# uci-cbcl/esm-efficient

Measured on AMD Instinct MI355X. Metric: residues/sec ESM2-650M fwd, 50k packed tokens; % bf16 MFMA peak; 1/2/4/8 GPU, higher is better.
Workload: dtype bf16

## Files before the change

### esm-efficient_amd/csrc/gemm.hip

```cpp
#include "gemm.h"
#ifndef ESME_GELU_PACKED
#define ESME_GELU_PACKED 1
#endif
#include <atomic>
#include <cstdlib>

#ifndef ESME_GEMM_P3N
#define ESME_GEMM_P3N 4
#endif
#ifndef ESME_GEMM_PERSIST_ROT
#define ESME_GEMM_PERSIST_ROT 0
#endif

namespace esme {

template <int BM, int BN, int WM, int WN, int EPI, int ROTD = 0, bool LNF = false, bool STATS = false, bool PERSIST = false, bool R32 = false, bool PAIR = false, bool F16 = false, bool RP = false>
__global__ __launch_bounds__(WM * WN * 64) void gemm_bf16_kernel(const GemmArgs a) {
    static_assert(!RP || (F16 && EPI == ESME_EPI_RESIDUAL && !R32 && !PAIR && !LNF && ROTD == 0), "pair stream: fp16 residual epilogue");
    static_assert(!F16 || ((!PAIR || (LNF && EPI == ESME_EPI_NONE)) && (EPI != ESME_EPI_RESIDUAL || R32 || RP)),
                  "fp16 operands: plain / GELU / SwiGLU epilogues, the fp32- / pair-stream residual epilogues, pair output of the LN-folded plain epilogue");
    static_assert(!LNF || EPI != ESME_EPI_RESIDUAL, "LN fold applies to the consumers of a LayerNorm");
    static_assert(!R32 || EPI == ESME_EPI_RESIDUAL, "the fp32 residual stream belongs to the residual epilogue");
    static_assert(!PAIR || (EPI != ESME_EPI_RESIDUAL && (!LNF || F16) && !STATS && !PERSIST), "(hi, lo) pair output: plain / GELU / SwiGLU epilogues of the split-operand mode; fp16: the LN-folded plain epilogue");
    static_assert(!STATS || (EPI == ESME_EPI_RESIDUAL && WTN_OK(BN, WN) && BN / WN == 64 && (WN == 2 || WN == 4)), "row statistics are emitted by the residual epilogue");
    static_assert(ROTD == 0 || (EPI == ESME_EPI_NONE && (ROTD == 16 || ROTD == 32 || ROTD == 64) && WTN_OK(BN, WN)),
                  "fused rotary: plain epilogue, head dim 16/32/64, 64-column wave tiles");
    constexpr int NW = WM * WN;
    constexpr int NT = NW * 64;
    constexpr int WTM = BM / WM, WTN = BN / WN;
    constexpr int FM = WTM / 16, FN = WTN / 16;
    constexpr int FMH = FM / 2;
    static_assert(FM % 2 == 0, "wave tile rows split in two halves");
    constexpr int A_ROWS_BYTES = BM * 128, W_ROWS_BYTES = BN * 128;
    constexpr int STAGE = A_ROWS_BYTES + W_ROWS_BYTES;
    constexpr int IA = BM * 8 / NT, IW = BN * 8 / NT;
    static_assert(BM * 8 % NT == 0 && BN * 8 % NT == 0, "tile/threads mismatch");
    static_assert(EPI != ESME_EPI_SWIGLU || WTN == 64, "swiglu needs 64-wide wave tiles");

    extern __shared__ __attribute__((aligned(16))) char smem[];
    constexpr int LDS_BYTES = 2 * (BM + BN) * 128 + ((LNF || ROTD > 0) ? BM * 12 + BN * 8 : 0) + (STATS ? WN * BM * 8 : 0) + (RP ? 2 * BN * 8 : 0);
    (void)LDS_BYTES;

    const int tid = threadIdx.x;
    const int lane = tid & 63;
    const int wave = __builtin_amdgcn_readfirstlane(tid >> 6);
    constexpr bool P8 = (NW == 8 && WM == 2 && WN == 4 && BM == 256 && BN == 256);
    const int wm = P8 ? (wave >> 2) : wave % WM, wn = P8 ? (wave & 3) : wave / WM;
    const int l15 = lane & 15, lq = lane >> 4;
    ESME_TRACE_REAL(8);
    ESME_TRACE_MARK(0);

#ifdef ESME_GEMM_TRACE
    if (a.stagger > 0 && blockIdx.x < 256) {
        const int n = (blockIdx.x * a.stagger) >> 8;
        for (int i = 0; i < n; ++i) __builtin_amdgcn_s_sleep(16);
    }
#endif
    unsigned int pid, pid_end = 0u, pid_step = 0u;
    if constexpr (PERSIST) {
        const unsigned int nblk = (unsigned int)(a.tiles_m * a.tiles_n);
        const unsigned int q = nblk >> 3, r = nblk & 7u, xcd = blockIdx.x & 7u, slot = blockIdx.x >> 3;
        const unsigned int base = (xcd < r) ? xcd * (q + 1) : r * (q + 1) + (xcd - r) * q;
        pid_step = gridDim.x >> 3;
        pid = base + slot;
        pid_end = base + q + (xcd < r ? 1u : 0u);
        if (pid >= pid_end) return;
    } else {
        pid = xcd_remap(blockIdx.x, gridDim.x);
    }
    int64_t m0;
    int n0;
    auto tile_coords = [&](const unsigned int id) {
        const int per_band = a.gm * a.tiles_n;
        const int band = id / per_band, lb = id - band * per_band;
        const int rows = min(a.gm, a.tiles_m - band * a.gm);
        const int grp = rows * a.gn;
        const int ng = lb / grp, rg = lb - ng * grp;
        const int tile_n = ng * a.gn + rg / rows;
        const int64_t tile_m = (int64_t)band * a.gm + rg % rows;
        m0 = tile_m * BM;
        n0 = tile_n * BN;
    };
    tile_coords(pid);

    const u16* srcA[IA];
    const u16* srcW[IW];
    auto set_sources = [&]() {
        int ln = lane;
        if constexpr (PERSIST) asm volatile("" : "+v"(ln));
#pragma unroll
        for (int i = 0; i < IA; ++i) {
            const int q = (i * NW + wave) * 64 + ln;
            const int row = q >> 3, c = (q & 7) ^ ((row >> 1) & 7);
            const int trow = P8 ? ((row >> 6) & 1) * WTM + (row >> 7) * (WTM / 2) + (row & 63) : row;
            int64_t gr = m0 + trow;
            gr = gr < a.M ? gr : a.M - 1;
            srcA[i] = a.A + gr * a.lda + c * 8;
        }
#pragma unroll
        for (int i = 0; i < IW; ++i) {
            const int q = (i * NW + wave) * 64 + ln;
            const int row = q >> 3, c = (q & 7) ^ ((row >> 1) & 7);
            const int tcol = P8 ? ((row >> 5) & 3) * WTN + (row >> 7) * (WTN / 2) + (row & 31) : row;
            int gr = n0 + tcol;
            gr = gr < a.N ? gr : a.N - 1;
            srcW[i] = a.W + (int64_t)gr * (a.kt_wrap > 0 ? a.kt_wrap * BK : a.K) + c * 8;
        }
    };
    set_sources();

    auto w_k0 = [&](const int kt) { return ((a.kt_wrap > 0 && kt >= a.kt_wrap) ? kt - a.kt_wrap : kt) * BK; };
    auto stage = [&](int kt, int buf) {
        char* base = smem + buf * STAGE;
        const int k0 = kt * BK, k0w = w_k0(kt);
#pragma unroll
        for (int i = 0; i < IA; ++i)
            __builtin_amdgcn_global_load_lds((gptr_t)(srcA[i] + k0), (lptr_t)(base + (i * NW + wave) * 1024), 16, 0, 0);
#pragma unroll
        for (int i = 0; i < IW; ++i)
            __builtin_amdgcn_global_load_lds((gptr_t)(srcW[i] + k0w),
                                             (lptr_t)(base + A_ROWS_BYTES + (i * NW + wave) * 1024), 16, 0, 0);
    };

    const int swz = (l15 >> 1) & 7;
    int coff[2];
#pragma unroll
    for (int ks = 0; ks < 2; ++ks) coff[ks] = ((ks * 4 + lq) ^ swz) << 4;
    const int rowA = (P8 ? wm * (WTM / 2) + l15 : wm * WTM + l15) * 128;
    const int rowW = A_ROWS_BYTES + (P8 ? wn * (WTN / 2) + l15 : wn * WTN + l15) * 128;

    f32x4 acc[FN][FM];
#pragma unroll
    for (int i = 0; i < FN; ++i)
#pragma unroll
        for (int j = 0; j < FM; ++j)
#pragma unroll
            for (int r = 0; r < 4; ++r) acc[i][j][r] = 0.f;

    const int KT = a.K / BK;
    struct FragW { bf16x8 v[FN]; };
    struct FragA { bf16x8 v[FMH]; };
    auto rdW = [&](FragW& f, const char* base, int ks) {
#pragma unroll
        for (int i = 0; i < FN; ++i) f.v[i] = *reinterpret_cast<const bf16x8*>(base + rowW + i * 16 * 128 + coff[ks]);
    };
    auto rdA = [&](FragA& f, const char* base, int ks, int h) {
#pragma unroll
        for (int j = 0; j < FMH; ++j) f.v[j] = *reinterpret_cast<const bf16x8*>(base + rowA + (h * FMH + j) * 16 * 128 + coff[ks]);
    };
    static_assert(IA % 2 == 0 && IW % 2 == 0, "the LDS-DMA pieces of a K-tile split in two halves");
    constexpr int NP = IA + IW;
    auto stage_piece = [&](int kt, int buf, int p) {
        char* base = smem + buf * STAGE;
        const int k0 = kt * BK;
        ESME_LDS_CHECK(p < IA ? base + (p * NW + wave) * 1024 : base + A_ROWS_BYTES + ((p - IA) * NW + wave) * 1024, 1024, smem, 2 * STAGE);
        if (p < IA) __builtin_amdgcn_global_load_lds((gptr_t)(srcA[p] + k0), (lptr_t)(base + (p * NW + wave) * 1024), 16, 0, 0);
        else __builtin_amdgcn_global_load_lds((gptr_t)(srcW[p - IA] + w_k0(kt)),
                                              (lptr_t)(base + A_ROWS_BYTES + ((p - IA) * NW + wave) * 1024), 16, 0, 0);
    };
    f32x2* lnst = reinterpret_cast<f32x2*>(smem + 2 * STAGE);
    int* lpos = reinterpret_cast<int*>(smem + 2 * STAGE + BM * 8);
    f32x4* c1s = reinterpret_cast<f32x4*>(smem + 2 * STAGE + BM * 12);
    f32x4* c2s = c1s + BN / 4;
    constexpr bool ROT32 = PAIR && ROTD > 0;
    constexpr int CPRW = ROTD > 0 ? (ROT32 ? ROTD / 4 : ROTD / 8) : 1;
    constexpr int TB = (ROT32 ? 4 : 2) * ROTD;
    constexpr int TAB_INSTR = WTM * CPRW / 64;
    constexpr int TAB_PER_WAVE = (TAB_INSTR + WN - 1) / WN;
    auto rot_prefetch = [&](int fb, int h) {
        if constexpr (ROTD > 0) {
            if (n0 >= a.rot_cols) return;
            char* tab = smem + fb * STAGE + wm * (WTM * TB);
#pragma unroll
            for (int it = 0; it < TAB_PER_WAVE; ++it) {
                if ((it & 1) != h && TAB_PER_WAVE > 1) continue;
                if (TAB_PER_WAVE == 1 && h != 0) continue;
                const int g = wn * TAB_PER_WAVE + it;
                if (g >= TAB_INSTR) continue;
                const int idx = g * 64 + lane;
                const int r = idx / CPRW;
                const int c = (idx % CPRW) ^ (r & (CPRW - 1));
                const int p = lpos[wm * WTM + r];
                const void* src;
                if constexpr (ROT32) src = (c < CPRW / 2) ? reinterpret_cast<const float*>(a.cosT) + (int64_t)p * ROTD + c * 4
                                                          : reinterpret_cast<const float*>(a.sinT) + (int64_t)p * ROTD + (c - CPRW / 2) * 4;
                else src = (c < CPRW / 2) ? a.cosT + (int64_t)p * ROTD + c * 8
                                          : a.sinT + (int64_t)p * ROTD + (c - CPRW / 2) * 8;
                ESME_LDS_CHECK(tab + g * 1024, 1024, smem, 2 * STAGE);
                __builtin_amdgcn_global_load_lds((gptr_t)src, (lptr_t)(tab + g * 1024), 16, 0, 0);
            }
        }
    };
    f32x4* pscale = reinterpret_cast<f32x4*>(smem + 2 * STAGE + (STATS ? WN * BM * 8 : 0));
    int sp = 0;
    auto fill_scales = [&](const int half) {
        if constexpr (RP) {
            if (tid < BN / 4) {
                int n = n0 + tid * 4;
                n = n < a.N - 4 ? n : a.N - 4;
                const f32x4 one = {1.f, 1.f, 1.f, 1.f};
                ESME_LDS_CHECK(&pscale[half * (BN / 2) + BN / 4 + tid], 16, smem, LDS_BYTES);
                pscale[half * (BN / 2) + tid] = a.ps_in ? *reinterpret_cast<const f32x4*>(a.ps_in + n) : one;
                pscale[half * (BN / 2) + BN / 4 + tid] = a.ps_out ? *reinterpret_cast<const f32x4*>(a.ps_out + n) : one;
            }
        }
    };
    int par = 0;
    stage(0, 0);
    auto make_strips = [&]() {
        if constexpr (ROTD > 0) {
            if (tid < BM) {
                int64_t m = m0 + tid;
                m = m < a.M ? m : a.M - 1;
                int p = a.pos[m];
                lpos[tid] = p < a.max_len ? p : a.max_len - 1;
            }
        }
        if constexpr (LNF) {
            if (tid < BM) {
                int64_t m = m0 + tid;
                m = m < a.M ? m : a.M - 1;
                float s1 = 0.f, s2 = 0.f;
                const f32x2* pp = reinterpret_cast<const f32x2*>(a.ln_partial) + m;
                const int n256 = (a.K + 255) >> 8;
                if (a.ln_nblk > n256) {
                    int b = 0;
                    for (; b + 10 <= a.ln_nblk; b += 10) {
                        f32x2 p[10];
    #pragma unroll
                        for (int u = 0; u < 10; ++u) p[u] = pp[(int64_t)(b + u) * a.stat_ld];
    #pragma unroll
                        for (int u = 0; u < 10; u += 2) { s1 += p[u][0] + p[u + 1][0]; s2 += p[u][1] + p[u + 1][1]; }
                    }
                    for (; b + 2 <= a.ln_nblk; b += 2) {
                        const f32x2 p0 = pp[(int64_t)b * a.stat_ld], p1 = pp[(int64_t)(b + 1) * a.stat_ld];
                        s1 += p0[0] + p1[0]; s2 += p0[1] + p1[1];
                    }
                    if (b < a.ln_nblk) { const f32x2 p = pp[(int64_t)b * a.stat_ld]; s1 += p[0]; s2 += p[1]; }
                } else {
                    int b = 0;
                    for (; b + 10 <= a.ln_nblk; b += 10) {
                        f32x2 p[10];
    #pragma unroll
                        for (int u = 0; u < 10; ++u) p[u] = pp[(int64_t)(b + u) * a.stat_ld];
    #pragma unroll
                        for (int u = 0; u < 10; ++u) { s1 += p[u][0]; s2 += p[u][1]; }
                    }
                    for (; b + 5 <= a.ln_nblk; b += 5) {
                        f32x2 p[5];
    #pragma unroll
                        for (int u = 0; u < 5; ++u) p[u] = pp[(int64_t)(b + u) * a.stat_ld];
    #pragma unroll
                        for (int u = 0; u < 5; ++u) { s1 += p[u][0]; s2 += p[u][1]; }
                    }
                    for (; b < a.ln_nblk; ++b) {
                        const f32x2 p = pp[(int64_t)b * a.stat_ld];
                        s1 += p[0]; s2 += p[1];
                    }
                }
                if (a.ovf && !(s2 < 3.0e38f)) atomicOr(a.ovf, 1);
                const float inv = 1.0f / (float)a.ln_dim;
                const float mean = s1 * inv;
                const float rstd = rsqrtf(fmaxf(s2 * inv - mean * mean, 0.f) + a.ln_eps);
                ESME_LDS_CHECK(&lnst[tid], 8, smem, LDS_BYTES);
                lnst[tid] = f32x2{rstd, rstd * mean};
            }
            if (tid < BN / 4) {
                int n = n0 + tid * 4;
                n = n < a.N - 4 ? n : a.N - 4;
                ESME_LDS_CHECK(&c2s[tid], 16, smem, LDS_BYTES);
                c1s[tid] = *reinterpret_cast<const f32x4*>(a.ln_c1 + n);
                c2s[tid] = *reinterpret_cast<const f32x4*>(a.ln_c2 + n);
            }
        }

    };
    make_strips();
    fill_scales(0);
    __syncthreads();
    FragW w0;
    FragA a0, a1;
#ifdef ESME_GEMM_TRACE
    unsigned long long trace_barrier_wait = 0, trace_vm_wait = 0;
    int trace_tile = -1;
#endif
    for (;;) {
    ESME_TRACE_MARK(1);
#ifdef ESME_GEMM_TRACE
    ++trace_tile;
#endif
    if constexpr (PERSIST) set_sources();
    if constexpr (P8) {
    if (KT > 1) {
        stage_piece(1, par ^ 1, IA); stage_piece(1, par ^ 1, IA + 1);
        stage_piece(1, par ^ 1, 0); stage_piece(1, par ^ 1, 1);
        stage_piece(1, par ^ 1, IA + 2); stage_piece(1, par ^ 1, IA + 3);
    }
    ESME_TRACE_SEAM(27, 2);
    if (wm == 1) __builtin_amdgcn_s_barrier();
    bf16x8 fa[FMH][2], fw[FN][2];
    constexpr int HALFB = (BM / 2) * 128;
    static_assert(FN == 4 && FMH == 4, "P8 geometry");
    auto rdW2 = [&](const char* base) {
#pragma unroll
        for (int i = 0; i < FN; ++i)
#pragma unroll
            for (int ks = 0; ks < 2; ++ks) {
                ESME_LDS_CHECK(base + rowW + (i >> 1) * HALFB + (i & 1) * 16 * 128 + coff[ks], 16, smem, 2 * STAGE);
                fw[i][ks] = *reinterpret_cast<const bf16x8*>(base + rowW + (i >> 1) * HALFB + (i & 1) * 16 * 128 + coff[ks]);
            }
    };
    auto rdAh = [&](const char* base, const int h) {
#pragma unroll
        for (int f = 0; f < FMH; ++f)
#pragma unroll
            for (int ks = 0; ks < 2; ++ks) {
                ESME_LDS_CHECK(base + rowA + h * HALFB + f * 16 * 128 + coff[ks], 16, smem, 2 * STAGE);
                fa[f][ks] = *reinterpret_cast<const bf16x8*>(base + rowA + h * HALFB + f * 16 * 128 + coff[ks]);
            }
    };
    auto mma = [&](const int j0) {
        asm volatile("s_waitcnt lgkmcnt(0)" ::: "memory");
        __builtin_amdgcn_sched_barrier(0);
        __builtin_amdgcn_s_barrier();
        __builtin_amdgcn_sched_barrier(0);
#pragma unroll
        for (int ks = 0; ks < 2; ++ks)
#pragma unroll
            for (int i = 0; i < FN; ++i)
#pragma unroll
                for (int f = 0; f < FMH; ++f)
                    acc[i][j0 + f] = mfma_16x16x32<F16>(fw[i][ks], fa[f][ks], acc[i][j0 + f]);
        __builtin_amdgcn_sched_barrier(0);
        __builtin_amdgcn_s_barrier();
        __builtin_amdgcn_sched_barrier(0);
    };
    for (int kt = 0; kt < KT; ++kt) {
        const int buf = (kt + par) & 1;
        const char* base = smem + buf * STAGE;
        const bool m1 = kt + 1 < KT, m2 = kt + 2 < KT;
        rdW2(base);
        rdAh(base, 0);
        if (m1) { stage_piece(kt + 1, buf ^ 1, 2); stage_piece(kt + 1, buf ^ 1, 3); }
        else rot_prefetch(buf ^ 1, 0);
        if (kt == 0) ESME_TRACE_SEAM(28, 2);
        mma(0);
        if (kt == 0) ESME_TRACE_SEAM(29, 2);
        rdAh(base, 1);
        if (m2) {
            stage_piece(kt + 2, buf, IA); stage_piece(kt + 2, buf, IA + 1);
            stage_piece(kt + 2, buf, 0); stage_piece(kt + 2, buf, 1);
            stage_piece(kt + 2, buf, IA + 2); stage_piece(kt + 2, buf, IA + 3);
        } else if (!m1) rot_prefetch(buf ^ 1, 1);
#ifdef ESME_GEMM_TRACE
        const unsigned long long bw0 = __builtin_readcyclecounter();
#endif
        if (m2) asm volatile("s_waitcnt vmcnt(6)" ::: "memory");
        else asm volatile("s_waitcnt vmcnt(0)" ::: "memory");
#ifdef ESME_GEMM_TRACE
        trace_vm_wait += __builtin_readcyclecounter() - bw0;
#endif
        mma(FMH);
    }
    ESME_TRACE_SEAM(16, 1);
    if (wm == 0) __builtin_amdgcn_s_barrier();
    ESME_TRACE_SEAM(17, 1);
    } else {
    rdW(w0, smem + par * STAGE, 0);
    rdA(a0, smem + par * STAGE, 0, 0);
    constexpr int P3 = (NP * ESME_GEMM_P3N) / 8;
    static_assert(FMH >= 2, "activation reads need FMH - 1 of every FMH MFMA slots");
    using std::integral_constant;
    auto sub = [&](FragW& w, const FragA& ca, auto H, auto NEWW, FragA& na, const char* nbase, const int nks,
                   const int nh, const bool rd_on, const bool on, const int kt, const int buf, auto PF, auto PL) {
        constexpr int h = decltype(H)::value, pf = decltype(PF)::value, pl = decltype(PL)::value, cnt = pl - pf, total = FN * FMH;
        constexpr bool neww = decltype(NEWW)::value;
        int na_next = 0;
#pragma unroll
        for (int m = 0; m < total; ++m) {
            const int i = m / FMH, j = m % FMH;
            acc[i][h * FMH + j] = mfma_16x16x32<F16>(w.v[i], ca.v[j], acc[i][h * FMH + j]);
            if (neww && j == FMH - 1) {
                if (rd_on) { ESME_LDS_CHECK(nbase + rowW + i * 16 * 128 + coff[nks], 16, smem, 2 * STAGE); w.v[i] = *reinterpret_cast<const bf16x8*>(nbase + rowW + i * 16 * 128 + coff[nks]); }
            } else if (na_next < FMH) {
                if (rd_on) { ESME_LDS_CHECK(nbase + rowA + (nh * FMH + na_next) * 16 * 128 + coff[nks], 16, smem, 2 * STAGE); na.v[na_next] = *reinterpret_cast<const bf16x8*>(nbase + rowA + (nh * FMH + na_next) * 16 * 128 + coff[nks]); }
                ++na_next;
            }
#pragma unroll
            for (int q = 0; q < (cnt > 0 ? cnt : 0); ++q)
                if (m == (q * total) / (cnt > 0 ? cnt : 1) && on) stage_piece(kt, buf, pf + q);
            __builtin_amdgcn_sched_barrier(0);
        }
    };
    using I0 = integral_constant<int, 0>; using I1 = integral_constant<int, 1>;
    using YES = integral_constant<bool, true>; using NO = integral_constant<bool, false>;
    if (KT > 1) {
#pragma unroll
        for (int p = 0; p < P3; ++p) stage_piece(1, par ^ 1, p);
    }
    for (int kt = 0; kt < KT; ++kt) {
        const int buf = (kt + par) & 1;
        const char* base = smem + buf * STAGE;
        const bool more = kt + 1 < KT, more2 = kt + 2 < KT;
        if (!more) rot_prefetch(buf ^ 1, 0);
        __builtin_amdgcn_sched_barrier(0);
        sub(w0, a0, I0{}, NO{}, a1, base, 0, 1, true, more, kt + 1, buf ^ 1, integral_constant<int, P3>{}, integral_constant<int, NP>{});
        if (!more) rot_prefetch(buf ^ 1, 1);
        __builtin_amdgcn_sched_barrier(0);
        sub(w0, a1, I1{}, YES{}, a0, base, 1, 0, true, false, 0, 0, I0{}, I0{});
        sub(w0, a0, I0{}, NO{}, a1, base, 1, 1, true, false, 0, 0, I0{}, I0{});
#ifdef ESME_GEMM_TRACE
        const unsigned long long bw0 = __builtin_readcyclecounter();
        asm volatile("s_waitcnt vmcnt(0) lgkmcnt(0)" ::: "memory");
        const unsigned long long bw1 = __builtin_readcyclecounter();
        trace_vm_wait += bw1 - bw0;
#endif
        __syncthreads();
#ifdef ESME_GEMM_TRACE
        trace_barrier_wait += __builtin_readcyclecounter() - bw1;
#endif
        __builtin_amdgcn_sched_barrier(0);
        sub(w0, a1, I1{}, YES{}, a0, smem + (buf ^ 1) * STAGE, 0, 0, more, more2, kt + 2, buf, I0{}, integral_constant<int, P3>{});
    }
    }
    ESME_TRACE_MARK(2);
#ifdef ESME_GEMM_TRACE
    if (a.trace && threadIdx.x == 0) { a.trace[(size_t)blockIdx.x * ESME_TRACE_STRIDE + 10] = trace_barrier_wait; a.trace[(size_t)blockIdx.x * ESME_TRACE_STRIDE + 11] = trace_vm_wait; }
#endif
#ifdef ESME_GEMM_TRACE
    if (a.nt_store == 3) return;
#endif

    int lane_e = threadIdx.x & 63;
    asm volatile("" : "+v"(lane_e));
    const int l15 = lane_e & 15, lq = lane_e >> 4, lane = lane_e;
    constexpr int OUTC = (EPI == ESME_EPI_SWIGLU) ? WTN / 2 : WTN;
    constexpr int CH = OUTC / 8;
    constexpr int ROWB = OUTC * 2;
    constexpr int RPI = 64 / CH;
    constexpr int NPASS = RP ? (BM == 256 ? 4 : 1)
                             : ((R32 && BM == 256) ? 4 : ((PERSIST || (PAIR && BM == 256)) ? 2 : 1));
    constexpr int RPP = WTM / NPASS;
    constexpr int FMP = FM / NPASS;
    static_assert(!PERSIST || (FM % 2 == 0), "two-pass epilogue");
    const int lastbuf = (a.K / BK - 1 + par) & 1;
    char* slab = smem + (PERSIST ? lastbuf * STAGE : 0) + wave * (RPP * ROWB) * (RP ? 2 : 1);
    const int64_t em0 = m0;
    const int en0 = n0;
    const int n_out = (EPI == ESME_EPI_SWIGLU) ? (a.N >> 1) : a.N;
    const int nw0 = (EPI == ESME_EPI_SWIGLU) ? ((n0 + wn * WTN) >> 1) : (n0 + wn * WTN);
    const int64_t mw0 = m0 + wm * WTM;
    auto slab_off = [&](const int r, const int cl) { return r * ROWB + (((cl >> 3) ^ (r & (CH - 1))) << 4) + (((cl >> 2) & 1) << 3); };

    if constexpr (LNF) {
        f32x2 st[FM];
#pragma unroll
        for (int j = 0; j < FM; ++j) st[j] = lnst[wm * WTM + j * 16 + l15];
#pragma unroll
        for (int i = 0; i < FN; ++i) {
            const int q4 = (wn * WTN + i * 16 + 4 * lq) >> 2;
            const f32x4 c1q = c1s[q4], c2q = c2s[q4];
#pragma unroll
            for (int j = 0; j < FM; ++j) {
#pragma unroll
                for (int e = 0; e < 4; ++e)
                    acc[i][j][e] = fmaf(st[j][0], acc[i][j][e], fmaf(-st[j][1], c1q[e], c2q[e]));
            }
        }
    }

    if constexpr (ROTD > 0) {
#pragma unroll
        for (int i = 0; i < FN; ++i) {
            if (LNF || !a.bias) continue;
            const u32x2 bw = *reinterpret_cast<const u32x2*>(a.bias + nw0 + i * 16 + 4 * lq);
            const float b0 = bf_lo(bw[0]), b1 = bf_hi(bw[0]), b2 = bf_lo(bw[1]), b3 = bf_hi(bw[1]);
#pragma unroll
            for (int j = 0; j < FM; ++j) {
                acc[i][j][0] += b0; acc[i][j][1] += b1; acc[i][j][2] += b2; acc[i][j][3] += b3;
            }
        }
        const char* tab = smem + (lastbuf ^ 1) * STAGE + wm * (WTM * TB);
        if (nw0 < a.rot_cols) {
#pragma unroll
            for (int j = 0; j < FM; ++j) {
                const int r = j * 16 + l15;
                const char* trow = tab + r * TB + (ROT32 ? 0 : (lq & 1) * 8);
                if constexpr (ROTD == 16) {
                    float cv[4], sv[4];
                    if constexpr (ROT32) {
                        const f32x4 cq = *reinterpret_cast<const f32x4*>(trow + (((lq & 1) ^ (r & 3)) << 4));
                        const f32x4 sq = *reinterpret_cast<const f32x4*>(trow + (((2 + (lq & 1)) ^ (r & 3)) << 4));
#pragma unroll
                        for (int e = 0; e < 4; ++e) { cv[e] = cq[e]; sv[e] = sq[e]; }
                    } else {
                        const u32x2 cw = *reinterpret_cast<const u32x2*>(trow + ((0 ^ (r & 1)) << 4));
                        const u32x2 sw = *reinterpret_cast<const u32x2*>(trow + ((1 ^ (r & 1)) << 4));
                        cv[0] = lo16<F16>(cw[0]); cv[1] = hi16<F16>(cw[0]); cv[2] = lo16<F16>(cw[1]); cv[3] = hi16<F16>(cw[1]);
// ... 289 lines not shown
#pragma unroll
                        for (int e = 0; e < 4; ++e) o[e] = gelu_erf<GELU_DEG>(o[e]);
#endif
                    }
                    if constexpr (R32) {
                        const int n = nw0 + cl;
                        const int64_t m = mw0 + pass * RPP + r;
#pragma unroll
                        for (int e = 0; e < 4; ++e) o[e] = fmaf(a.alpha, o[e], xr[i][jj][e]);
                        if (m < a.M && n < a.N) store_stream(reinterpret_cast<f32x4*>(a.resid32 + m * a.ld32 + n), f32x4{o[0], o[1], o[2], o[3]}, a.stream_out);
                    } else if constexpr (EPI == ESME_EPI_RESIDUAL) {
                        const u32x2 rw = *reinterpret_cast<const u32x2*>(slab + slab_off(r, cl));
                        o[0] = bf_lo(rw[0]) + a.alpha * o[0]; o[1] = bf_hi(rw[0]) + a.alpha * o[1];
                        o[2] = bf_lo(rw[1]) + a.alpha * o[2]; o[3] = bf_hi(rw[1]) + a.alpha * o[3];
                    }
                }
                u32x2 pk = {pack16<F16>(o[0], o[1]), pack16<F16>(o[2], o[3])};
                if (PAIR && half == 0) {
                    acc[i][j][0] = o[0] - lo16<F16>(pk[0]); acc[i][j][1] = o[1] - hi16<F16>(pk[0]);
                    acc[i][j][2] = o[2] - lo16<F16>(pk[1]); acc[i][j][3] = o[3] - hi16<F16>(pk[1]);
                }
                ESME_LDS_CHECK(slab + slab_off(r, cl), 8, smem, 2 * STAGE);
                *reinterpret_cast<u32x2*>(slab + slab_off(r, cl)) = pk;
            }
            if constexpr (EPI == ESME_EPI_RESIDUAL && !R32) __builtin_amdgcn_sched_barrier(0);
        }
        if (pass + 1 < NPASS && half == NHALF - 1) load_x32(pass + 1);
        __builtin_amdgcn_wave_barrier();
        ESME_TRACE_MARK(5);
        if constexpr (PERSIST) {
            if (pass == NPASS / 2 - 1) {
                ESME_TRACE_SEAM(19, 1);
                __syncthreads();
                ESME_TRACE_SEAM(20, 1);
                pid += pid_step;
                have_next = pid < pid_end;
                if (have_next) {
                    tile_coords(pid);
                    set_sources();
                    par = lastbuf ^ 1;
                    stage(0, par);
                    make_strips();
                }
                ESME_TRACE_SEAM(21, 1);
            }
        }
        if constexpr (PERSIST) {
            if (pass == 0) ESME_TRACE_SEAM(31, 1);
            if (pass == NPASS - 1) ESME_TRACE_SEAM(23, 1);
            if (pass == NPASS - 1 && have_next) asm volatile("s_waitcnt vmcnt(0)" ::: "memory");
            if (pass == NPASS - 1) ESME_TRACE_SEAM(24, 1);
        }
        const int rl = lane / CH, ch = lane % CH;
        const int n = nw0 + ch * 8;
        const bool col_ok = n < n_out && !(PAIR && half == 1 && a.pair_cols > 0 && en0 >= a.pair_cols);
        constexpr bool QKG = F16 && LNF && ROTD > 0 && !PAIR;
        const bool qk_guard = QKG && a.qk_sumsq != nullptr && nw0 < a.rot_cols;
        float qk_max = 0.f;
        unsigned int* qk_slot = nullptr;
        unsigned int qk_cur = 0u;
        if constexpr (QKG) {
            if (qk_guard && lane < 8 && (n % ROTD) == 0 && n < a.rot_cols) {
                const int ea = a.rot_cols >> 1;
                qk_slot = a.qk_sumsq + (n >= ea ? ea / ROTD : 0) + (n % ea) / ROTD;
                qk_cur = *qk_slot;
            }
        }
        if (col_ok || STATS) {
#pragma unroll
        for (int gsel = 0; gsel < (QKG ? 2 : 1); ++gsel) {
            if (QKG && (gsel == 1) != qk_guard) continue;
#pragma unroll
            for (int it = 0; it < RPP / RPI; ++it) {
                const int r = it * RPI + rl;
                const int64_t m = mw0 + pass * RPP + r;
                ESME_LDS_CHECK(slab + r * ROWB + ((ch ^ (r & (CH - 1))) << 4), 16, smem, 2 * STAGE);
                const u32x4 v = *reinterpret_cast<const u32x4*>(slab + r * ROWB + ((ch ^ (r & (CH - 1))) << 4));
                if (col_ok && m < a.M && ESME_TUNE_STORE_OK) store_stream(reinterpret_cast<u32x4*>(a.C + m * a.ldc + n + (PAIR ? half * a.pair_off : 0)), v, a.stream_out);
                if (QKG && gsel == 1) {
                    float ss = sumsq8_f16(v);
                    ss += dpp_f32<0xB1>(ss);
                    if constexpr (ROTD >= 32) ss += dpp_f32<0x4E>(ss);
                    if constexpr (ROTD == 64) ss += dpp_f32<0x141>(ss);
                    qk_max = fmaxf(qk_max, ss);
                }
                if constexpr (STATS) {
                    float f[8];
                    unpack8t<F16>(v, f);
                    float t1 = ((f[0] + f[1]) + (f[2] + f[3])) + ((f[4] + f[5]) + (f[6] + f[7]));
                    float t2 = ((f[0] * f[0] + f[1] * f[1]) + (f[2] * f[2] + f[3] * f[3])) +
                               ((f[4] * f[4] + f[5] * f[5]) + (f[6] * f[6] + f[7] * f[7]));
                    t1 += dpp_f32<0xB1>(t1); t2 += dpp_f32<0xB1>(t2);
                    t1 += dpp_f32<0x4E>(t1); t2 += dpp_f32<0x4E>(t2);
                    t1 += dpp_f32<0x141>(t1); t2 += dpp_f32<0x141>(t2);
                    ESME_LDS_CHECK(&blkst[wn * BM + wm * WTM + pass * RPP + r], 8, smem, LDS_BYTES);
                    if (ch == 0) blkst[wn * BM + wm * WTM + pass * RPP + r] = col_ok ? f32x2{t1, t2} : f32x2{0.f, 0.f};
                }
            }
        }
        }
        if constexpr (QKG) {
            if (qk_guard) {
                qk_max = lanes8_max_f32(qk_max);
                if (qk_slot && __float_as_uint(qk_max) > qk_cur) atomicMax(qk_slot, __float_as_uint(qk_max));
            }
        }
        if constexpr (PERSIST) { if (pass == 0) ESME_TRACE_SEAM(22, 1); else ESME_TRACE_SEAM(25, 1); }
        }
        }
        }
        ESME_TRACE_MARK(6);
        if constexpr (STATS) {
            asm volatile("s_waitcnt lgkmcnt(0)" ::: "memory");
            __builtin_amdgcn_s_barrier();
            if (tid < BM && em0 + tid < a.M) {
                f32x2 acc2 = blkst[tid];
                acc2[0] += blkst[BM + tid][0]; acc2[1] += blkst[BM + tid][1];
                if constexpr (WN == 4) {
                    f32x2 hi2 = blkst[2 * BM + tid];
                    hi2[0] += blkst[3 * BM + tid][0]; hi2[1] += blkst[3 * BM + tid][1];
                    acc2[0] += hi2[0]; acc2[1] += hi2[1];
                }
                *reinterpret_cast<f32x2*>(a.stats_out + 2 * ((int64_t)(en0 / BN) * a.stat_ld + em0 + tid)) = acc2;
            }
        }
        ESME_TRACE_MARK(7);
        ESME_TRACE_REAL(9);
    } else {
        if constexpr (EPI != ESME_EPI_SWIGLU) {
    #pragma unroll
            for (int i = 0; i < FN; ++i) {
                const int n = nw0 + i * 16 + 4 * lq;
    #pragma unroll
                for (int j = 0; j < FM; ++j) {
                    const int64_t m = mw0 + j * 16 + l15;
                    if (m >= a.M) continue;
    #pragma unroll
                    for (int e = 0; e < 4; ++e) {
                        if (n + e < a.N) {
                            float v = acc[i][j][e] + ((a.bias && ROTD == 0 && !LNF) ? bf2f(a.bias[n + e]) : 0.f);
                            if constexpr (EPI == ESME_EPI_GELU) v = gelu_erf<LNF ? ESME_GELU_DEG : 7>(v);
                            if constexpr (R32) { float* xp = a.resid32 + m * a.ld32 + n + e; v = fmaf(a.alpha, v, *xp); *xp = v; }
                            else if constexpr (EPI == ESME_EPI_RESIDUAL) v = bf2f(a.resid[m * a.ldr + n + e]) + a.alpha * v;
                            if (a.c32) a.c32[m * a.ldc32 + n + e] = v;
                            else a.C[m * a.ldc + n + e] = f2h<F16>(v);
                        }
                    }
                }
            }
        }
    }
    if constexpr (!PERSIST) {
        break;
    } else {
        if (!have_next) break;
#pragma unroll
        for (int i = 0; i < FN; ++i)
#pragma unroll
            for (int j = 0; j < FM; ++j)
#pragma unroll
                for (int r = 0; r < 4; ++r) acc[i][j][r] = 0.f;
        asm volatile("s_waitcnt lgkmcnt(0)" ::: "memory");
        ESME_TRACE_SEAM(26, 1);
        __builtin_amdgcn_s_barrier();
    }
    }
}
// ... 91 lines not shown
                    case 32: return lnf ? ESME_LH(ESME_EPI_NONE, 32, true, false, false) : fail(ESME_ERR_UNSUPPORTED, "gemm: fp16 fused rotary runs LayerNorm-folded only");
                    case 64: return lnf ? ESME_LH(ESME_EPI_NONE, 64, true, false, false) : fail(ESME_ERR_UNSUPPORTED, "gemm: fp16 fused rotary runs LayerNorm-folded only");
                    default: return fail(ESME_ERR_UNSUPPORTED, "gemm: fused rotary needs head dim 16, 32 or 64");
                }
            case ESME_EPI_GELU: return lnf ? ESME_LH(ESME_EPI_GELU, 0, true, false, false) : ESME_LH(ESME_EPI_GELU, 0, false, false, false);
            case ESME_EPI_SWIGLU: return lnf ? ESME_LH(ESME_EPI_SWIGLU, 0, true, false, false) : fail(ESME_ERR_UNSUPPORTED, "gemm: fp16 SwiGLU runs LayerNorm-folded only");
            case ESME_EPI_RESIDUAL:
                if (a.pair_off)
                    return stats ? launch_one<BM, BN, WM, WN, ESME_EPI_RESIDUAL, 0, false, true, false, false, false, true, true>(a, s)
                                 : launch_one<BM, BN, WM, WN, ESME_EPI_RESIDUAL, 0, false, false, false, false, false, true, true>(a, s);
                return stats ? ESME_LH(ESME_EPI_RESIDUAL, 0, false, true, true) : ESME_LH(ESME_EPI_RESIDUAL, 0, false, false, true);
            default: return fail(ESME_ERR_ARG, "gemm: unknown epilogue");
        }
#undef ESME_LH
    }
    switch (epi) {
        case ESME_EPI_NONE:
            switch (rotd) {
                case 0: return lnf ? ESME_L(ESME_EPI_NONE, 0, true, false) : ESME_L(ESME_EPI_NONE, 0, false, false);
                case 16: return lnf ? ESME_L(ESME_EPI_NONE, 16, true, false) : ESME_L(ESME_EPI_NONE, 16, false, false);
                case 32: return lnf ? ESME_L(ESME_EPI_NONE, 32, true, false) : ESME_L(ESME_EPI_NONE, 32, false, false);
                case 64: return lnf ? ESME_L(ESME_EPI_NONE, 64, true, false) : ESME_L(ESME_EPI_NONE, 64, false, false);
                default: return fail(ESME_ERR_UNSUPPORTED, "gemm: fused rotary needs head dim 16, 32 or 64");
            }
        case ESME_EPI_GELU: return lnf ? ESME_L(ESME_EPI_GELU, 0, true, false) : ESME_L(ESME_EPI_GELU, 0, false, false);
        case ESME_EPI_SWIGLU: return lnf ? ESME_L(ESME_EPI_SWIGLU, 0, true, false) : ESME_L(ESME_EPI_SWIGLU, 0, false, false);
        case ESME_EPI_RESIDUAL:
            if (a.resid32) return stats ? launch_one<BM, BN, WM, WN, ESME_EPI_RESIDUAL, 0, false, true, false, true>(a, s)
                                        : launch_one<BM, BN, WM, WN, ESME_EPI_RESIDUAL, 0, false, false, false, true>(a, s);
            return stats ? ESME_L(ESME_EPI_RESIDUAL, 0, false, true) : ESME_L(ESME_EPI_RESIDUAL, 0, false, false);
        default: return fail(ESME_ERR_ARG, "gemm: unknown epilogue");
    }
#undef ESME_L
}

}

using namespace esme;

static int esme::cu_count() {
    static std::atomic<int> cached[64];
    int dev = 0;
    (void)hipGetDevice(&dev);
    int v = cached[dev & 63].load(std::memory_order_relaxed);
    if (v <= 0) {
        if (hipDeviceGetAttribute(&v, hipDeviceAttributeMultiprocessorCount, dev) != hipSuccess || v <= 0) v = 256;
        cached[dev & 63].store(v, std::memory_order_relaxed);
    }
    return v;
}
#ifdef ESME_GEMM_TRACE
extern "C" void esme_hip_debug_set_gemm_nt(int v) { esme::g_nt_store = v; }
extern "C" void esme_hip_debug_set_gemm_stagger(int v) { esme::g_stagger = v; }
static unsigned long long* g_trace = nullptr;
extern "C" void esme_hip_debug_set_gemm_trace(void* p) { g_trace = (unsigned long long*)p; }
#endif

static int pick_tile(int64_t M, int N, const esme_gemm_opts_t* opts) {
    if (opts && opts->tile) return opts->tile;
    const int64_t big_tiles = ((M + 255) / 256) * ((N + 255) / 256);
    return (N >= 256 && big_tiles >= 160) ? 2 : 1;
}

extern "C" int esme_hip_gemm_stats_blocks_opts(int64_t M, int N, const esme_gemm_opts_t* opts) {
    const int bn = pick_tile(M, N, opts) == 2 ? 256 : 128;
    return (N + bn - 1) / bn;
}
extern "C" int esme_hip_gemm_stats_blocks(int64_t M, int N) { return esme_hip_gemm_stats_blocks_opts(M, N, nullptr); }

extern "C" int esme_hip_gemm_bf16_opts(const void* A, int64_t lda, const void* W, const void* bias, const void* resid,
                                       int64_t ldr, void* C, int64_t ldc, int64_t M, int N, int K, int epilogue,
                                       float alpha, const esme_gemm_fusion_t* fu, const esme_gemm_opts_t* opts, void* stream) {
    ESME_CHECK_ARG(!opts || (opts->struct_bytes == (int)sizeof(esme_gemm_opts_t) && opts->tile >= 0 && opts->tile <= 2),
                   "gemm: options struct of another ABI or bad tile");
    ESME_CHECK_ARG(M >= 0 && N > 0 && K > 0, "gemm: bad sizes");
    ESME_CHECK_ARG(epilogue >= ESME_EPI_NONE && epilogue <= ESME_EPI_SWIGLU, "gemm: unknown epilogue");
    if (M == 0) return ESME_OK;
    ESME_CHECK_ARG(A && W && C, "gemm: null pointer");
    if (K % BK != 0) ESME_FAIL(ESME_ERR_UNSUPPORTED, "gemm: K must be a multiple of 64");
    const int n_out = epilogue == ESME_EPI_SWIGLU ? N / 2 : N;
    if (epilogue == ESME_EPI_SWIGLU && N % 64 != 0) ESME_FAIL(ESME_ERR_UNSUPPORTED, "gemm: swiglu needs N % 64 == 0");
    ESME_CHECK_ARG(lda >= K && lda % 8 == 0 && ldc >= n_out, "gemm: bad lda/ldc");
    ESME_CHECK_ARG(aligned16(A) && aligned16(W), "gemm: A and W must be 16-byte aligned");
    ESME_CHECK_ARG(!bias || (reinterpret_cast<uintptr_t>(bias) & 7u) == 0, "gemm: misaligned bias");
    int vec_ok = (ldc % 8 == 0) && aligned16(C) && (n_out % 8 == 0) && N >= 8;
    const bool r32 = fu && fu->resid32;
    if (r32) {
        ESME_CHECK_ARG(epilogue == ESME_EPI_RESIDUAL, "gemm: resid32 belongs to the residual epilogue");
        ESME_CHECK_ARG(fu->ld32 >= N && fu->ld32 % 4 == 0 && aligned16(fu->resid32), "gemm: resid32 needs ld32 >= N, ld32 % 4 == 0, 16-byte alignment");
        if (!vec_ok) ESME_FAIL(ESME_ERR_UNSUPPORTED, "gemm: the fp32 residual stream needs a 16-byte addressable C and N % 8 == 0");
    } else if (epilogue == ESME_EPI_RESIDUAL) {
        ESME_CHECK_ARG(resid && ldr >= N, "gemm: residual epilogue needs resid with ldr >= N");
        vec_ok = vec_ok && (ldr % 8 == 0) && aligned16(resid) && N >= 8;
    }
    if (epilogue == ESME_EPI_SWIGLU && !vec_ok) ESME_FAIL(ESME_ERR_UNSUPPORTED, "gemm: swiglu needs ldc % 8 == 0 and a 16-byte aligned C");
    GemmArgs a{(const u16*)A, lda, (const u16*)W, (const u16*)bias, (const u16*)resid, ldr, (u16*)C, ldc, M, N, K, alpha, 0, vec_ok,
               nullptr, nullptr, nullptr, 0, 0, 0, 1, 1, 0, 0, nullptr, 0, 0, 0.f, nullptr, nullptr, nullptr};
#ifdef ESME_GEMM_TRACE
    a.nt_store = g_nt_store; a.stagger = g_stagger; a.trace = g_trace;
#endif
    if (opts) { a.opt_gm = opts->raster_gm; a.opt_gn = opts->raster_gn; a.opt_persist = opts->persist; }
    int rotd = 0;
    bool lnf = false, stats = false;
    if (r32) { a.resid32 = fu->resid32; a.ld32 = fu->ld32; }
    ESME_CHECK_ARG(!fu || (!fu->pair_scale_in && !fu->pair_scale_out && !fu->ext_off) || (fu->f16 && fu->pair_off && epilogue == ESME_EPI_RESIDUAL),
                   "gemm: pair_scale_in / pair_scale_out / ext_* belong to the fp16 pair stream's residual epilogue");
    ESME_CHECK_ARG(!fu || !fu->pair_cols || (fu->f16 && fu->pair_off && epilogue == ESME_EPI_NONE), "gemm: pair_cols belongs to the fp16 pair output");
    ESME_CHECK_ARG(!fu || !fu->col_absmax || (fu->f16 && fu->pair_off && epilogue == ESME_EPI_RESIDUAL), "gemm: col_absmax belongs to the fp16 pair stream's residual epilogue");
    ESME_CHECK_ARG(!fu || !fu->qk_sumsq || (fu->f16 && fu->ln_partial && fu->head_dim != 0 && !fu->pair_off), "gemm: qk_sumsq belongs to the fp16 LN-folded projection with fused rotary (single output)");
    if (fu && fu->f16 && fu->pair_off && epilogue == ESME_EPI_NONE) {
        ESME_CHECK_ARG(fu->ln_partial && !r32 && !fu->w_k && !fu->c32 && !fu->stats_out, "gemm: the fp16 pair output belongs to the LN-folded plain epilogue");
        ESME_CHECK_ARG(fu->pair_off >= N && fu->pair_off % 8 == 0 && ldc >= fu->pair_off + (fu->pair_cols > 0 ? fu->pair_cols : N) && fu->pair_cols >= 0 && fu->pair_cols % 256 == 0,
                       "gemm: pair_off must be a multiple of 8 with N <= pair_off and room for the lo columns; pair_cols a multiple of 256");
        if (!vec_ok) ESME_FAIL(ESME_ERR_UNSUPPORTED, "gemm: pair output needs a 16-byte addressable C and N % 8 == 0");
        a.pair_off = fu->pair_off; a.pair_cols = fu->pair_cols;
    } else if (fu && fu->f16 && fu->pair_off) {
        ESME_CHECK_ARG(epilogue == ESME_EPI_RESIDUAL && !r32 && !fu->w_k && !fu->c32 && !fu->ln_partial, "gemm: the fp16 pair stream belongs to the residual epilogue");
        ESME_CHECK_ARG(fu->pair_off >= N && fu->pair_off % 8 == 0 && ldc >= fu->pair_off + N && ldr >= fu->pair_off + N,
                       "gemm: pair_off must be a multiple of 8 with N <= pair_off <= ldc - N, ldr - N");
        if (!vec_ok) ESME_FAIL(ESME_ERR_UNSUPPORTED, "gemm: the pair stream needs 16-byte addressable rows and N % 8 == 0");
        a.pair_off = fu->pair_off;
        ESME_CHECK_ARG((!fu->pair_scale_in || aligned16(fu->pair_scale_in)) && (!fu->pair_scale_out || aligned16(fu->pair_scale_out)) && (N % 4 == 0),
                       "gemm: pair_scale_in / pair_scale_out must be 16-byte aligned float (N) vectors");
        a.ps_in = fu->pair_scale_in; a.ps_out = fu->pair_scale_out;
        if (fu->ext_off) {
            ESME_CHECK_ARG(fu->ext_off >= N && fu->ext_off + 64 <= fu->pair_off && fu->ext_n >= 0 && fu->ext_n <= 64 && (fu->ext_n == 0 || fu->ext_sel),
                           "gemm: the extension tile is 64 columns between hi and lo (N <= ext_off, ext_off + 64 <= pair_off) with <= 64 selected columns");
            a.ext_sel = fu->ext_sel; a.ext_n = fu->ext_n; a.ext_off = fu->ext_off;
        }
        ESME_CHECK_ARG(!fu->col_absmax || (reinterpret_cast<uintptr_t>(fu->col_absmax) & 3u) == 0, "gemm: misaligned col_absmax");
        a.col_absmax = fu->col_absmax;
    } else if (fu && (fu->w_k || fu->pair_off || fu->c32)) {
        if (fu->w_k) {
            ESME_CHECK_ARG(fu->w_k > 0 && fu->w_k % BK == 0 && (K == fu->w_k || K == 2 * fu->w_k), "gemm: w_k (the K of W) must be a multiple of 64 with K = w_k or K = 2 w_k (the K-tile index of W wraps once)");
            if (fu->w_k < K) a.kt_wrap = fu->w_k / BK;
        }
        if (fu->pair_off) {
            ESME_CHECK_ARG(epilogue != ESME_EPI_RESIDUAL && !fu->ln_partial && !fu->stats_out, "gemm: pair output belongs to the plain / GELU / SwiGLU epilogues without LN fold");
            ESME_CHECK_ARG(fu->pair_off >= n_out && fu->pair_off % 8 == 0 && ldc >= fu->pair_off + n_out, "gemm: pair_off must be a multiple of 8 with n_out <= pair_off <= ldc - n_out");
            if (!vec_ok) ESME_FAIL(ESME_ERR_UNSUPPORTED, "gemm: pair output needs a 16-byte addressable C and N % 8 == 0");
            a.pair_off = fu->pair_off;
        }
        if (fu->c32) {
            ESME_CHECK_ARG(!fu->pair_off && epilogue != ESME_EPI_SWIGLU && fu->ldc32 >= N && (reinterpret_cast<uintptr_t>(fu->c32) & 3u) == 0, "gemm: c32 needs ldc32 >= N, no pair output, no SwiGLU");
            a.c32 = fu->c32; a.ldc32 = fu->ldc32;
            a.vec_ok = 0;
        }
    }
    if (fu && fu->f16) {
        ESME_CHECK_ARG(!fu->w_k && !fu->c32 && (!fu->pair_off || epilogue == ESME_EPI_RESIDUAL || epilogue == ESME_EPI_NONE), "gemm: fp16 operands do not combine with the split-operand fields");
        ESME_CHECK_ARG(epilogue != ESME_EPI_RESIDUAL || r32 || fu->pair_off, "gemm: fp16 operands run the residual epilogue on the fp32 stream or the fp16 pair stream");
        if (!vec_ok) ESME_FAIL(ESME_ERR_UNSUPPORTED, "gemm: fp16 operands need a 16-byte addressable C and N % 8 == 0");
        a.f16 = 1;
    }
    if (fu) {
        if (fu->head_dim != 0) {
            ESME_CHECK_ARG(epilogue == ESME_EPI_NONE, "gemm: fused rotary needs ESME_EPI_NONE");
            ESME_CHECK_ARG(fu->cos && fu->sin && fu->pos && fu->max_len > 0, "gemm: fused rotary needs cos, sin, pos, max_len");
            if (fu->head_dim != 16 && fu->head_dim != 32 && fu->head_dim != 64)
                ESME_FAIL(ESME_ERR_UNSUPPORTED, "gemm: fused rotary needs head dim 16, 32 or 64 (use esme_hip_rotary_varlen otherwise)");
            if (N % 64 != 0 || fu->rot_cols % 64 != 0 || fu->rot_cols < 0 || fu->rot_cols > N || !vec_ok)
                ESME_FAIL(ESME_ERR_UNSUPPORTED, "gemm: fused rotary needs N, rot_cols multiples of 64, rot_cols <= N, 16-byte addressable C");
            ESME_CHECK_ARG(aligned16(fu->cos) && aligned16(fu->sin), "gemm: misaligned rotary tables");
            ESME_CHECK_ARG(!fu->pair_off || fu->q_scale == 0.f, "gemm: q_scale does not combine with a pair output");
            a.cosT = (const u16*)fu->cos; a.sinT = (const u16*)fu->sin; a.pos = fu->pos;
            a.max_len = fu->max_len; a.rot_cols = fu->rot_cols;
// ... 88 lines not shown
```

Baseline: 826,800.

## Stage GEMM tiles with buffer_load LDS DMA using scalar row offsets

Result: slower. 817,400, median of 2 (-1.1%).

```diff
diff --git a/esm-efficient_amd/csrc/gemm.hip b/esm-efficient_amd/csrc/gemm.hip
--- a/esm-efficient_amd/csrc/gemm.hip
+++ b/esm-efficient_amd/csrc/gemm.hip
@@ -3,6 +3,7 @@
 #define ESME_GELU_PACKED 1
 #endif
 #include <atomic>
+#include <type_traits>
 #include <cstdlib>
 
 #ifndef ESME_GEMM_P3N
@@ -83,43 +84,59 @@
     };
     tile_coords(pid);
 
-    const u16* srcA[IA];
-    const u16* srcW[IW];
+    static_assert(NW % 2 == 0, "chunk swizzle independent of the piece index");
+    const unsigned int ldA = (unsigned int)a.lda * 2u, ldW = (unsigned int)(a.kt_wrap > 0 ? a.kt_wrap * BK : a.K) * 2u;
+    unsigned int voffA, voffW;
+    {
+        const unsigned int r = (unsigned int)lane >> 3, c = ((unsigned int)lane & 7u) ^ ((((unsigned int)wave & 1u) << 2) + ((unsigned int)lane >> 4));
+        voffA = r * ldA + c * 16u;
+        voffW = r * ldW + c * 16u;
+    }
+    auto rowA_of = [&](const int i) { return P8 ? (i & 1) * WTM + (i >> 1) * (WTM / 2) + wave * 8 : (i * NW + wave) * 8; };
+    auto rowW_of = [&](const int i) { return P8 ? ((i & 1) * 2 + (wave >> 2)) * WTN + (i >> 1) * (WTN / 2) + (wave & 3) * 8 : (i * NW + wave) * 8; };
+    auto make_rsrc = [&](const u16* p, const unsigned int bytes) -> u32x4 {
+        const uint64_t v = (uint64_t)(uintptr_t)p;
+        return u32x4{(unsigned int)__builtin_amdgcn_readfirstlane((int)(unsigned int)v),
+                     (unsigned int)__builtin_amdgcn_readfirstlane((int)((unsigned int)(v >> 32) & 0xffffu)),
+                     (unsigned int)__builtin_amdgcn_readfirstlane((int)bytes), 0x00020000u};
+    };
+    u32x4 rsA, rsW;
     auto set_sources = [&]() {
-        int ln = lane;
-        if constexpr (PERSIST) asm volatile("" : "+v"(ln));
-#pragma unroll
-        for (int i = 0; i < IA; ++i) {
-            const int q = (i * NW + wave) * 64 + ln;
-            const int row = q >> 3, c = (q & 7) ^ ((row >> 1) & 7);
-            const int trow = P8 ? ((row >> 6) & 1) * WTM + (row >> 7) * (WTM / 2) + (row & 63) : row;
-            int64_t gr = m0 + trow;
-            gr = gr < a.M ? gr : a.M - 1;
-            srcA[i] = a.A + gr * a.lda + c * 8;
-        }
-#pragma unroll
-        for (int i = 0; i < IW; ++i) {
-            const int q = (i * NW + wave) * 64 + ln;
-            const int row = q >> 3, c = (q & 7) ^ ((row >> 1) & 7);
-            const int tcol = P8 ? ((row >> 5) & 3) * WTN + (row >> 7) * (WTN / 2) + (row & 31) : row;
-            int gr = n0 + tcol;
-            gr = gr < a.N ? gr : a.N - 1;
-            srcW[i] = a.W + (int64_t)gr * (a.kt_wrap > 0 ? a.kt_wrap * BK : a.K) + c * 8;
-        }
+        const int64_t mrows = a.M - m0;
+        const unsigned int vm = mrows < BM ? (unsigned int)mrows : (unsigned int)BM;
+        const int ncols = a.N - n0;
+        const unsigned int vn = ncols < BN ? (unsigned int)ncols : (unsigned int)BN;
+        rsA = make_rsrc(a.A + m0 * a.lda, (vm - 1u) * ldA + (unsigned int)a.K * 2u);
+        rsW = make_rsrc(a.W + (int64_t)n0 * (ldW >> 1), vn * ldW);
     };
     set_sources();
+    auto dma16 = [&](const u32x4 rs, const unsigned int voff, const unsigned int soff, const char* dst, auto FRESH) {
+        const unsigned int d = (unsigned int)__builtin_amdgcn_readfirstlane((int)(unsigned int)(uintptr_t)dst);
+        const unsigned int so = (unsigned int)__builtin_amdgcn_readfirstlane((int)soff);
+        const u32x4 r = {(unsigned int)__builtin_amdgcn_readfirstlane((int)rs[0]), (unsigned int)__builtin_amdgcn_readfirstlane((int)rs[1]),
+                         (unsigned int)__builtin_amdgcn_readfirstlane((int)rs[2]), 0x00020000u};
+        unsigned int keep;
+#if defined(ESME_DEBUG_LDS) || defined(ESME_GEMM_TRACE)
+        constexpr bool pad = true;
+#else
+        constexpr bool pad = decltype(FRESH)::value;
+#endif
+        if constexpr (pad)
+            asm volatile("s_nop 4\n\ts_mov_b32 %0, m0\n\ts_mov_b32 m0, %2\n\ts_nop 0\n\tbuffer_load_dwordx4 %1, %3, %4 offen lds\n\ts_mov_b32 m0, %0"
+                         : "=&s"(keep) : "v"(voff), "s"(d), "s"(r), "s"(so) : "memory");
+        else
+            asm volatile("s_mov_b32 %0, m0\n\ts_mov_b32 m0, %2\n\ts_nop 0\n\tbuffer_load_dwordx4 %1, %3, %4 offen lds\n\ts_mov_b32 m0, %0"
+                         : "=&s"(keep) : "v"(voff), "s"(d), "s"(r), "s"(so) : "memory");
+    };
 
     auto w_k0 = [&](const int kt) { return ((a.kt_wrap > 0 && kt >= a.kt_wrap) ? kt - a.kt_wrap : kt) * BK; };
     auto stage = [&](int kt, int buf) {
         char* base = smem + buf * STAGE;
-        const int k0 = kt * BK, k0w = w_k0(kt);
-#pragma unroll
-        for (int i = 0; i < IA; ++i)
-            __builtin_amdgcn_global_load_lds((gptr_t)(srcA[i] + k0), (lptr_t)(base + (i * NW + wave) * 1024), 16, 0, 0);
-#pragma unroll
-        for (int i = 0; i < IW; ++i)
-            __builtin_amdgcn_global_load_lds((gptr_t)(srcW[i] + k0w),
-                                             (lptr_t)(base + A_ROWS_BYTES + (i * NW + wave) * 1024), 16, 0, 0);
+        const unsigned int k0 = (unsigned int)(kt * BK) * 2u, k0w = (unsigned int)w_k0(kt) * 2u;
+#pragma unroll
+        for (int i = 0; i < IA; ++i) dma16(rsA, voffA, (unsigned int)rowA_of(i) * ldA + k0, base + (i * NW + wave) * 1024, std::true_type{});
+#pragma unroll
+        for (int i = 0; i < IW; ++i) dma16(rsW, voffW, (unsigned int)rowW_of(i) * ldW + k0w, base + A_ROWS_BYTES + (i * NW + wave) * 1024, std::true_type{});
     };
 
     const int swz = (l15 >> 1) & 7;
@@ -152,11 +169,9 @@
     constexpr int NP = IA + IW;
     auto stage_piece = [&](int kt, int buf, int p) {
         char* base = smem + buf * STAGE;
-        const int k0 = kt * BK;
         ESME_LDS_CHECK(p < IA ? base + (p * NW + wave) * 1024 : base + A_ROWS_BYTES + ((p - IA) * NW + wave) * 1024, 1024, smem, 2 * STAGE);
-        if (p < IA) __builtin_amdgcn_global_load_lds((gptr_t)(srcA[p] + k0), (lptr_t)(base + (p * NW + wave) * 1024), 16, 0, 0);
-        else __builtin_amdgcn_global_load_lds((gptr_t)(srcW[p - IA] + w_k0(kt)),
-                                              (lptr_t)(base + A_ROWS_BYTES + ((p - IA) * NW + wave) * 1024), 16, 0, 0);
+        if (p < IA) dma16(rsA, voffA, (unsigned int)rowA_of(p) * ldA + (unsigned int)(kt * BK) * 2u, base + (p * NW + wave) * 1024, std::false_type{});
+        else dma16(rsW, voffW, (unsigned int)rowW_of(p - IA) * ldW + (unsigned int)w_k0(kt) * 2u, base + A_ROWS_BYTES + ((p - IA) * NW + wave) * 1024, std::false_type{});
     };
     f32x2* lnst = reinterpret_cast<f32x2*>(smem + 2 * STAGE);
     int* lpos = reinterpret_cast<int*>(smem + 2 * STAGE + BM * 8);
@@ -277,6 +292,7 @@
     };
     make_strips();
     fill_scales(0);
+    asm volatile("s_waitcnt vmcnt(0)" ::: "memory");
     __syncthreads();
     FragW w0;
     FragA a0, a1;
@@ -289,7 +305,6 @@
 #ifdef ESME_GEMM_TRACE
     ++trace_tile;
 #endif
-    if constexpr (PERSIST) set_sources();
     if constexpr (P8) {
     if (KT > 1) {
         stage_piece(1, par ^ 1, IA); stage_piece(1, par ^ 1, IA + 1);
@@ -414,6 +429,8 @@
         asm volatile("s_waitcnt vmcnt(0) lgkmcnt(0)" ::: "memory");
         const unsigned long long bw1 = __builtin_readcyclecounter();
         trace_vm_wait += bw1 - bw0;
+#else
+        asm volatile("s_waitcnt vmcnt(0)" ::: "memory");
 #endif
         __syncthreads();
 #ifdef ESME_GEMM_TRACE
@@ -869,7 +886,7 @@
                     ss += dpp_f32<0xB1>(ss);
                     if constexpr (ROTD >= 32) ss += dpp_f32<0x4E>(ss);
                     if constexpr (ROTD == 64) ss += dpp_f32<0x141>(ss);
-                    qk_max = fmaxf(qk_max, ss);
+                    qk_max = fmaxf(qk_max, m < a.M ? ss : 0.f);
                 }
                 if constexpr (STATS) {
                     float f[8];
@@ -1127,6 +1144,7 @@
     if (epilogue == ESME_EPI_SWIGLU && N % 64 != 0) ESME_FAIL(ESME_ERR_UNSUPPORTED, "gemm: swiglu needs N % 64 == 0");
     ESME_CHECK_ARG(lda >= K && lda % 8 == 0 && ldc >= n_out, "gemm: bad lda/ldc");
     ESME_CHECK_ARG(aligned16(A) && aligned16(W), "gemm: A and W must be 16-byte aligned");
+    if (lda > (int64_t)0x7fffff || K > 0x7fffff) ESME_FAIL(ESME_ERR_UNSUPPORTED, "gemm: row strides of 2^23 elements or more are not supported");
     ESME_CHECK_ARG(!bias || (reinterpret_cast<uintptr_t>(bias) & 7u) == 0, "gemm: misaligned bias");
     int vec_ok = (ldc % 8 == 0) && aligned16(C) && (n_out % 8 == 0) && N >= 8;
     const bool r32 = fu && fu->resid32;
```
